# petabi/petal-neighbors

Measured on NVIDIA B200. Metric: knn_queries_per_sec_k10, higher is better.
Workload: dtype f32

## Files before the change

### petal-neighbors_b200/csrc/engine.cu

```cuda
#include <sys/mman.h>

#include <chrono>
#include <condition_variable>
#include <cstdio>
#include <cstdlib>
#include <memory>
#include <atomic>
#include <mutex>
#include <string>
#include <vector>

#include "../../include/petal_b200.h"
#include "flat_tree.hpp"
#include "comm.hpp"
#include "gpu_build.hpp"
#include "kernels.cuh"
#include "tc_filter.cuh"

namespace petal {

static thread_local std::string g_err;
static int fail(int code, const std::string& msg) {
    g_err = msg;
    return code;
// ... 456 lines not shown
        TRY(hb.ensure(sizeof(h)));
        CU(cudaMemcpyAsync(hb.p, &h, sizeof(h), cudaMemcpyHostToDevice, cm->stream));
        NC(cm->api->Broadcast(hb.p, hb.p, sizeof(h), ncclUint8, root, cm->comm, cm->stream));
        for (auto& a : replica_arrays()) NC(cm->api->Broadcast(a.first->p, a.first->p, a.second, ncclUint8, root, cm->comm, cm->stream));
        CU(cudaStreamSynchronize(cm->stream));
        return PN_OK;
    }
    int replicate_recv(pn_comm* cm, int root) {
        device = cm->device;
        DeviceGuard g(device);
        if (!g.ok) return fail(PN_CUDA, "cudaSetDevice failed");
        ReplicaHeader h{};
        DevBuf hb;
        TRY(hb.ensure(sizeof(h)));
        NC(cm->api->Broadcast(hb.p, hb.p, sizeof(h), ncclUint8, root, cm->comm, cm->stream));
        CU(cudaMemcpyAsync(&h, hb.p, sizeof(h), cudaMemcpyDeviceToHost, cm->stream));
        CU(cudaStreamSynchronize(cm->stream));
        ft.n = h.n; ft.n_total = h.n_total; ft.d = h.d; ft.dpad = h.dpad; ft.L = h.L; ft.n_internal = h.n_internal; ft.n_buckets = h.n_buckets;
        ft.n_nodes = h.n_nodes; ft.bucket_max = h.bucket_max; ft.kind = h.kind; kp = h.kp; algo = h.algo; tensor_ready = h.tensor_ready != 0;
        pmax = h.pmax; tscale = h.tscale; prune_on = (h.prune_on & 1u) != 0; tiles_on = (h.prune_on & 2u) != 0;
        gpu_built = true;
        bytes = 0;
        for (auto& a : replica_arrays()) {
            TRY(a.first->ensure(a.second));
            NC(cm->api->Broadcast(a.first->p, a.first->p, a.second, ncclUint8, root, cm->comm, cm->stream));
            bytes += a.first->cap;
        }
        CU(cudaStreamSynchronize(cm->stream));
        ft.bucket_lo.resize(ft.n_buckets); ft.bucket_hi.resize(ft.n_buckets);
        CU(cudaMemcpy(ft.bucket_lo.data(), d_blo.p, (size_t)ft.n_buckets * 4, cudaMemcpyDeviceToHost));
        CU(cudaMemcpy(ft.bucket_hi.data(), d_bhi.p, (size_t)ft.n_buckets * 4, cudaMemcpyDeviceToHost));
        if (ft.kind == 1) {
            ft.vp_ids.resize(std::max<uint32_t>(ft.n_nodes, 1));
            CU(cudaMemcpy(ft.vp_ids.data(), d_vpids.p, ft.vp_ids.size() * 4, cudaMemcpyDeviceToHost));
        }
        fill_dev_tree();
        return PN_OK;
    }
};

template <typename A>
struct Engine final : pn_tree {
    using V = typename VT<A>::V;
    std::shared_ptr<DeviceTree<A>> tree;
    bool owns_tree = true;
    int n_sms = 148;
    cudaStream_t stream = nullptr, last_stream = nullptr;
    cudaEvent_t ev[4] = {nullptr, nullptr, nullptr, nullptr};
    DevBuf w_qraw, w_q, w_home, w_hist, w_cursor, w_order, w_part_d, w_part_i, w_floor_d, w_floor_i,
        w_counters, w_out_i, w_out_d, w_counts, w_offsets, w_hits;
    cudaStream_t s_in = nullptr, s_out = nullptr;
    cudaEvent_t e_in[2] = {nullptr, nullptr}, e_cmp[2] = {nullptr, nullptr}, e_out[2] = {nullptr, nullptr};
    DevBuf w_qraw2[2], w_oi2[2], w_od2[2];
    DevBuf sh_li[2], sh_ld[2], sh_pack[2], sh_gat[2], sh_gat_d[2];
    std::vector<cudaEvent_t> sh_ev;
    DevBuf r_qraw[2], r_q[2], r_counts[2], r_offsets[2], r_hits[2], r_slab[2], r_qlist[2], r_nlist[2], r_sums[2];
    unsigned long long* pin_tot = nullptr;
    void* pin_stage[2] = {nullptr, nullptr};
    cudaEvent_t pin_ev[2] = {nullptr, nullptr};
    static constexpr size_t PIN_BYTES = 16u << 20;
    DevBuf w_aaug, w_qmargin, w_trace, w_gbound;
    bool last_used_tensor = false;
    DevBuf w_qs, w_seed, w_bits, w_tcnt;
    DevBuf w_bcen, w_brad, w_bmu, w_qth, w_bbits, w_bcnt, w_wslot, w_wlist, w_wbits, w_nwide;
    bool last_pruned = false, last_tiles = false;

    explicit Engine(std::shared_ptr<DeviceTree<A>> t) : tree(std::move(t)) {}
    ~Engine() override {
        if (!host_only) {
            DeviceGuard g(tree->device);
            for (auto& e : ev) if (e) cudaEventDestroy(e);
            for (int i = 0; i < 2; ++i) {
                if (pin_stage[i]) cudaFreeHost(pin_stage[i]);
                if (pin_ev[i]) cudaEventDestroy(pin_ev[i]);
                for (cudaEvent_t e : {e_in[i], e_cmp[i], e_out[i]}) if (e) cudaEventDestroy(e);
            }
            for (cudaEvent_t e : sh_ev) cudaEventDestroy(e);
            if (pin_tot) cudaFreeHost(pin_tot);
            if (s_in) cudaStreamDestroy(s_in);
            if (s_out) cudaStreamDestroy(s_out);
            if (stream) cudaStreamDestroy(stream);
        }
    }

    int open_device() {
        DeviceGuard g(tree->device);
        if (!g.ok) return fail(PN_CUDA, "no usable CUDA device (there is no CPU fallback)");
        CU(cudaDeviceGetAttribute(&n_sms, cudaDevAttrMultiProcessorCount, tree->device));
        CU(cudaStreamCreateWithFlags(&stream, cudaStreamNonBlocking));
        for (auto& e : ev) CU(cudaEventCreate(&e));
        return PN_OK;
    }

    uint64_t device_bytes() const override {
        if (!owns_tree) return 0;
        const auto p = tree->partition();
        return tree->bytes + (p ? p->bytes : 0);
    }

    template <int DVR, int K, int KIND>
    int launch_knn_t(const DeviceTree<A>& t, const KnnArgs<A>& a, dim3 grid, cudaStream_t st) {
        size_t smem = DVR < 0 ? 0 : 2 * TILE_BYTES + (DVR == 0 ? (size_t)TQ * t.ft.dpad * sizeof(A) : 0);
        auto kern = knn_tile_kernel<A, DVR, K, KIND>;
        if (smem > 32 * 1024) CU(cudaFuncSetAttribute(kern, cudaFuncAttributeMaxDynamicSharedMemorySize, (int)smem));
        kern<<<grid, TQ, smem, st>>>(a);
        CU(cudaGetLastError());
        return PN_OK;
    }
    template <int K, int KIND>
    int launch_knn_k(const DeviceTree<A>& t, const KnnArgs<A>& a, dim3 grid, cudaStream_t st) {
        switch (t.dt.dv) {
            case 1: return launch_knn_t<1, K, KIND>(t, a, grid, st);
            case 2: return launch_knn_t<2, K, KIND>(t, a, grid, st);
            case 4: return launch_knn_t<4, K, KIND>(t, a, grid, st);
            case 8: return launch_knn_t<8, K, KIND>(t, a, grid, st);
            default:
                if ((size_t)t.ft.dpad * sizeof(A) > 1024) return launch_knn_t<-1, K, KIND>(t, a, grid, st);
                return launch_knn_t<0, K, KIND>(t, a, grid, st);
        }
    }
    int launch_knn(const DeviceTree<A>& t, const KnnArgs<A>& a, dim3 grid, cudaStream_t st, bool k1) {
        if (t.ft.kind == 0) return k1 ? launch_knn_k<1, 0>(t, a, grid, st) : launch_knn_k<16, 0>(t, a, grid, st);
        return k1 ? launch_knn_k<1, 1>(t, a, grid, st) : launch_knn_k<16, 1>(t, a, grid, st);
    }


    typedef CUresult (*EncodeTiledFn)(CUtensorMap*, CUtensorMapDataType, cuuint32_t, void*, const cuuint64_t*, const cuuint64_t*,
                                      const cuuint32_t*, const cuuint32_t*, CUtensorMapInterleave, CUtensorMapSwizzle,
                                      CUtensorMapL2promotion, CUtensorMapFloatOOBfill);
    static EncodeTiledFn encode_fn() {
        static EncodeTiledFn fn = [] {
            void* p = nullptr;
            cudaDriverEntryPointQueryResult q;
            if (cudaGetDriverEntryPoint("cuTensorMapEncodeTiled", &p, cudaEnableDefault, &q) != cudaSuccess) { (void)cudaGetLastError(); p = nullptr; }
            return (EncodeTiledFn)p;
        }();
        return fn;
    }
    static int make_map(CUtensorMap* m, void* base, uint64_t rows, uint32_t box_rows, uint32_t kp) {
        EncodeTiledFn fn = encode_fn();
        if (!fn) return fail(PN_CUDA, "cuTensorMapEncodeTiled entry point not found");
        cuuint64_t dims[2] = {kp, rows};
        cuuint64_t strides[1] = {(cuuint64_t)kp * 2};
        cuuint32_t box[2] = {(cuuint32_t)tc::KC, (cuuint32_t)box_rows};
        cuuint32_t estr[2] = {1, 1};
        CUresult r = fn(m, CU_TENSOR_MAP_DATA_TYPE_FLOAT16, 2, base, dims, strides, box, estr, CU_TENSOR_MAP_INTERLEAVE_NONE,
                        CU_TENSOR_MAP_SWIZZLE_64B, CU_TENSOR_MAP_L2_PROMOTION_L2_256B, CU_TENSOR_MAP_FLOAT_OOB_FILL_NONE);
        if (r != CUDA_SUCCESS) return fail(PN_CUDA, "cuTensorMapEncodeTiled failed with code " + std::to_string((int)r));
        return PN_OK;
    }
    static constexpr size_t filter_fixed_smem(int mt, uint32_t k) {
        return 1024 + 1024 + (size_t)4 * mt * 192 * 4 + (size_t)4 * mt * k * 32 * 8;
    }
    template <int DVR, int K, int MT, int NACC, int SW = tc::BN>
    int launch_filter_t(const DeviceTree<A>& t, const CUtensorMap& map_a, const tc::FilterArgs& fa, cudaStream_t st) {
        if (fa.tile_bits) return launch_filter_s<DVR, K, MT, NACC, false, SW, true>(t, map_a, fa, st);
        return fa.g_bound ? launch_filter_s<DVR, K, MT, NACC, true, SW, false>(t, map_a, fa, st) : launch_filter_s<DVR, K, MT, NACC, false, SW, false>(t, map_a, fa, st);
    }
    template <int DVR, int K, int MT, int NACC, bool SHARED, int SW, bool PRUNE>
    int launch_filter_s(const DeviceTree<A>& t, const CUtensorMap& map_a, const tc::FilterArgs& fa, cudaStream_t st) {
        const size_t smem = filter_fixed_smem(MT, fa.k) + (size_t)MT * fa.nkc * tc::A_CHUNK_BYTES + (size_t)fa.stages * fa.gs * tc::CHUNK_BYTES;
        auto kern = tc::knn_filter_kernel<DVR, K, MT, NACC, SHARED, SW, PRUNE>;
        CU(cudaFuncSetAttribute(kern, cudaFuncAttributeMaxDynamicSharedMemorySize, (int)smem));
        const unsigned gx = (fa.nq - fa.row0 + MT * tc::BM - 1) / (MT * tc::BM);
        const unsigned gy = PRUNE ? 1u : (fa.n_tiles + fa.tiles_per_split - 1) / fa.tiles_per_split;
        kern<<<dim3(gx, gy), (5 * MT + 2) * 32, smem, st>>>(map_a, t.d_baug.template as<unsigned char>(), fa);
        CU(cudaGetLastError());
        return PN_OK;
    }
    template <int K>
    int launch_filter_k(const DeviceTree<A>& t, const CUtensorMap& map_a, tc::FilterArgs& fa, cudaStream_t st) {
        const int mt = t.filter_subtiles(fa.nkc);
        const size_t budget = 224 * 1024;
        fa.gs = fa.nkc == 1 ? 2 : (fa.nkc == 2 ? 2 : 1);
        const size_t fixed = filter_fixed_smem(mt, fa.k) + (size_t)mt * fa.nkc * tc::A_CHUNK_BYTES;
        fa.stages = fixed < budget ? (uint32_t)std::min<size_t>(fa.gs > 1 ? 8 : 12, (budget - fixed) / (tc::CHUNK_BYTES * fa.gs)) : 0;
        fa.stages &= ~1u;
        if (fa.stages < 2) return fail(PN_CUDA, "tensor path: shared memory budget too small for this dimension");
        if (mt == 4) {
            bool half = fa.nkc == 1;
#ifdef PN_TC_PROFILE
            if (getenv("PN_TC_HALF")) half = atoi(getenv("PN_TC_HALF")) != 0;
#endif
            if (half) {
                if (t.dt.dv == 4) return launch_filter_t<4, K, 4, 2, 64>(t, map_a, fa, st);
                if (t.dt.dv == 8) return launch_filter_t<8, K, 4, 2, 64>(t, map_a, fa, st);
                return launch_filter_t<0, K, 4, 2, 64>(t, map_a, fa, st);
            }
            if (t.dt.dv == 4) return launch_filter_t<4, K, 4, 1>(t, map_a, fa, st);
            if (t.dt.dv == 8) return launch_filter_t<8, K, 4, 1>(t, map_a, fa, st);
            return launch_filter_t<0, K, 4, 1>(t, map_a, fa, st);
        }
#if defined(PN_TC_PROFILE) || defined(PN_TC_EXPERIMENTS)
        if (mt == 3) {
            if (fa.nkc == 1) return t.dt.dv == 4 ? launch_filter_t<4, K, 3, 2, 64>(t, map_a, fa, st) : launch_filter_t<0, K, 3, 2, 64>(t, map_a, fa, st);
            return launch_filter_t<0, K, 3, 1>(t, map_a, fa, st);
        }
#endif
        if (mt == 2) {
            if (t.dt.dv == 4) return launch_filter_t<4, K, 2, 2>(t, map_a, fa, st);
            if (t.dt.dv == 8) return launch_filter_t<8, K, 2, 2>(t, map_a, fa, st);
#if defined(PN_TC_PROFILE) || defined(PN_TC_EXPERIMENTS)
            {
                static const int ts = getenv("PN_TC_TS") ? atoi(getenv("PN_TC_TS")) : 0;
                if (ts == 1 && fa.nkc <= 8) return launch_filter_t<0, K, 2, 2, 64>(t, map_a, fa, st);
                if (ts == 2) return launch_filter_t<0, K, 2, 1>(t, map_a, fa, st);
            }
#endif
            return launch_filter_t<0, K, 2, 2>(t, map_a, fa, st);
        }
        return launch_filter_t<0, K, 1, 2>(t, map_a, fa, st);
    }

    int sort_and_seed(const DeviceTree<A>& t, const A* qraw, uint32_t nq, size_t stride, uint32_t k, cudaStream_t st, bool self_query, const float4** qsorted,
                      const uint32_t** order) {
        if constexpr (sizeof(A) == 4) {
            *order = nullptr;
            TRY(w_home.ensure((size_t)nq * 4));
            if (self_query) {
                TRY(w_hist.ensure((size_t)t.ft.n_buckets * 4));
                home_bucket_kernel<A><<<(nq + 127) / 128, 128, 0, st>>>(t.dt, t.d_pts.template as<V>(), nq, w_home.as<uint32_t>(), w_hist.as<uint32_t>());
                CU(cudaGetLastError());
                ++counters.kernel_launches;
                *qsorted = t.d_pts.template as<float4>();
            } else {
                TRY(stage_queries(t, qraw, nq, stride, st, true));
                TRY(w_qs.ensure((size_t)nq * t.ft.dpad * 4));
                const size_t tot = (size_t)nq * t.dt.dv;
                tc::gather_queries_kernel<<<(unsigned)((tot + 255) / 256), 256, 0, st>>>(w_q.as<float4>(), w_order.as<uint32_t>(), nq, t.dt.dv, w_qs.as<float4>());
                CU(cudaGetLastError());
                ++counters.kernel_launches;
                *qsorted = w_qs.as<float4>();
                *order = w_order.as<uint32_t>();
            }
            TRY(w_seed.ensure((size_t)nq * 4));
            const DevTree<float>& dtf = *reinterpret_cast<const DevTree<float>*>(&t.dt);
            tc::seed_bound_kernel<<<(nq + 7) / 8, 256, 0, st>>>(dtf, *qsorted, *order, w_home.as<uint32_t>(), nq, k, w_seed.as<float>());
            CU(cudaGetLastError());
            ++counters.kernel_launches;
            return PN_OK;
        } else {
            (void)qraw; (void)nq; (void)stride; (void)k; (void)st; (void)self_query; (void)qsorted; (void)order;
            return fail(PN_BAD_ARG, "the tensor path is f32 only");
        }
    }

    int knn_device_pruned(const DeviceTree<A>& t, const A* qraw, uint32_t nq, size_t stride, uint32_t k, uint32_t kstride, uint64_t* idx_out, A* dist_out, cudaStream_t st,
                          bool self_query) {
        if constexpr (sizeof(A) == 4) {
            const bool k1 = (k == 1);
            const uint32_t KP = k1 ? 1 : 16;
            const uint32_t n_tiles = (uint32_t)((t.ft.n + tc::BN - 1) / tc::BN), words = (n_tiles + 31) / 32;
            const uint32_t QT = 128u * (uint32_t)t.filter_subtiles(t.kp / tc::KC), n_qt = (nq + QT - 1) / QT;
            const float4* qsorted;
            const uint32_t* order = nullptr;
            CU(cudaEventRecord(ev[2], st));
            static const bool stage_timing = getenv("PN_STAGE_TIMING") != nullptr;
            cudaEvent_t se[5] = {nullptr, nullptr, nullptr, nullptr, nullptr};
            if (stage_timing) { for (auto& e : se) CU(cudaEventCreate(&e)); CU(cudaEventRecord(se[0], st)); }
            TRY(sort_and_seed(t, qraw, nq, stride, k, st, self_query, &qsorted, &order));
            if (stage_timing) CU(cudaEventRecord(se[1], st));
            TRY(w_aaug.ensure((size_t)nq * t.kp * 2));
            TRY(w_qmargin.ensure((size_t)nq * 4));
            TRY(w_bits.ensure((size_t)n_qt * words * 4));
            TRY(w_tcnt.ensure((size_t)n_qt * 4));
            TRY(w_part_d.ensure((size_t)nq * KP * 4));
            TRY(w_part_i.ensure((size_t)nq * KP * 4));
            const DevTree<float>& dtf = *reinterpret_cast<const DevTree<float>*>(&t.dt);
            tc::build_aaug_kernel<<<(nq + 127) / 128, 128, 0, st>>>(reinterpret_cast<const float*>(qsorted), t.d_center.template as<float>(), t.tscale, nq, t.ft.d, t.ft.dpad,
                                                                    t.kp, t.pmax, w_aaug.as<__half>(), w_qmargin.as<float>());
            CU(cudaGetLastError());
            {
                static const int wide_div = getenv("PN_WIDE_DIV") ? atoi(getenv("PN_WIDE_DIV")) : 4;
                const uint32_t n_sub = QT / 32, n_warps = n_qt * n_sub, n_balls = 2 * n_warps;
                const uint32_t wide_cap = wide_div > 0 ? std::max<uint32_t>(1u, n_warps / (uint32_t)wide_div) : 1u;
                const size_t smem = (size_t)32 * t.dt.dv * 16;
                TRY(w_bcen.ensure((size_t)n_balls * t.ft.dpad * 4)); TRY(w_brad.ensure((size_t)n_balls * 4)); TRY(w_bmu.ensure((size_t)n_balls * 4));
                TRY(w_qth.ensure((size_t)n_warps * 32 * 4)); TRY(w_bbits.ensure((size_t)n_balls * words * 4)); TRY(w_bcnt.ensure((size_t)n_balls * 4));
                TRY(w_wslot.ensure((size_t)n_warps * 4)); TRY(w_wlist.ensure((size_t)wide_cap * 4)); TRY(w_wbits.ensure((size_t)wide_cap * words * 4));
                TRY(w_nwide.ensure(4));
                if (smem > 48u * 1024u) {
                    CU(cudaFuncSetAttribute(tc::ball_tile_kernel<false>, cudaFuncAttributeMaxDynamicSharedMemorySize, (int)smem));
                    CU(cudaFuncSetAttribute(tc::ball_tile_kernel<true>, cudaFuncAttributeMaxDynamicSharedMemorySize, (int)smem));
                }
                CU(cudaMemsetAsync(w_nwide.p, 0, 4, st));
                tc::warp_balls_kernel<<<(n_warps + 7) / 8, 256, 0, st>>>(qsorted, w_seed.as<float>(), nq, n_warps, t.dt.dv, w_bcen.as<float4>(), w_brad.as<float>(),
                                                                         w_bmu.as<float>(), w_qth.as<float>());
                CU(cudaGetLastError());
                tc::ball_tile_kernel<false><<<(n_balls + 31) / 32, 256, smem, st>>>(w_bcen.as<float4>(), w_brad.as<float>(), w_bmu.as<float>(), n_balls, nullptr, nullptr, 0u,
                                                                                   t.d_tcen.template as<float>(), t.d_trad.template as<float>(), n_tiles, t.dt.dv, (float)t.dt.slack, words,
                                                                                   w_bbits.as<uint32_t>(), w_bcnt.as<uint32_t>());
                CU(cudaGetLastError());
                tc::wide_select_kernel<<<(n_qt + 127) / 128, 128, 0, st>>>(w_bcnt.as<uint32_t>(), w_bmu.as<float>(), n_qt, n_sub, wide_div > 0 ? wide_cap : 0u, w_wslot.as<uint32_t>(),
                                                                          w_wlist.as<uint32_t>(), w_nwide.as<uint32_t>());
                CU(cudaGetLastError());
                tc::ball_tile_kernel<true><<<wide_cap, 256, smem, st>>>(qsorted, nullptr, w_qth.as<float>(), nq, w_wlist.as<uint32_t>(), w_nwide.as<uint32_t>(), wide_div > 0 ? wide_cap : 0u,
                                                                       t.d_tcen.template as<float>(), t.d_trad.template as<float>(), n_tiles, t.dt.dv, (float)t.dt.slack, words,
                                                                       w_wbits.as<uint32_t>(), nullptr);
                CU(cudaGetLastError());
                tc::group_bits_kernel<<<n_qt, 256, 0, st>>>(w_bbits.as<uint32_t>(), w_wbits.as<uint32_t>(), w_wslot.as<uint32_t>(), nq, QT, n_sub, words,
                                                            w_bits.as<uint32_t>(), w_tcnt.as<uint32_t>(), w_counters.as<unsigned long long>() + 3);
                CU(cudaGetLastError());
                counters.kernel_launches += 4;
            }
            counters.kernel_launches += 2;
            if (stage_timing) CU(cudaEventRecord(se[2], st));
            alignas(64) CUtensorMap map_a;
            TRY(make_map(&map_a, w_aaug.p, nq, tc::BM, t.kp));
            tc::FilterArgs fa{};
            fa.t = dtf;
            fa.q = qsorted; fa.q_margin = w_qmargin.as<float>();
            fa.k = k; fa.n_tiles = n_tiles; fa.tiles_per_split = n_tiles;
            fa.nkc = t.kp / tc::KC;
            fa.last_steps = ((t.ft.d + tc::NSLOT - 1) % tc::KC) / 16 + 1;
            fa.t2_scale = t.tscale * t.tscale * (1.0f + (float)(t.ft.d + 4) * 1.1920928955078125e-07f);
            fa.part_d = w_part_d.as<float>(); fa.part_i = w_part_i.as<uint32_t>();
            fa.counters = w_counters.as<unsigned long long>();
            fa.row0 = 0; fa.nq = nq; fa.g_bound = nullptr;
            fa.tile_bits = w_bits.as<uint32_t>(); fa.tile_cnt = w_tcnt.as<uint32_t>(); fa.tile_words = words; fa.seed_t2 = w_seed.as<float>();
            TRY(k1 ? launch_filter_k<1>(t, map_a, fa, st) : launch_filter_k<16>(t, map_a, fa, st));
            if (stage_timing) CU(cudaEventRecord(se[3], st));
            CU(merge_lists<A, uint32_t>(st, w_part_d.as<A>(), w_part_i.as<uint32_t>(), 1, nq, k, idx_out, dist_out, kstride,
                                                                            0, nullptr, nullptr, self_query ? t.d_ids.template as<uint32_t>() : order));
            CU(cudaGetLastError());
            if (stage_timing) {
                CU(cudaEventRecord(se[4], st));
                CU(cudaEventSynchronize(se[4]));
                float t[4] = {0.f, 0.f, 0.f, 0.f};
                for (int i = 0; i < 4; ++i) (void)cudaEventElapsedTime(&t[i], se[i], se[i + 1]);
                fprintf(stderr, "[pn stage timing] pruned scan, %u queries, k %u: sort + seeds %.2f ms | operands + tile bitmaps %.2f ms | filter %.2f ms | merge %.2f ms\n",
                        nq, k, t[0], t[1], t[2], t[3]);
                for (auto& e : se) cudaEventDestroy(e);
            }
            counters.kernel_launches += 2;
            counters.filter_pairs += (uint64_t)t.ft.n * nq;
            CU(cudaEventRecord(ev[3], st));
            return PN_OK;
        } else {
            (void)qraw; (void)nq; (void)stride; (void)k; (void)kstride; (void)idx_out; (void)dist_out; (void)st; (void)self_query;
            return fail(PN_BAD_ARG, "the tensor path is f32 only");
// ... 1526 lines not shown
```

### petal-neighbors_b200/csrc/tc_filter.cuh

```cuda
#pragma once
#include <cuda.h>
#include <cuda_fp16.h>
#include <cuda_runtime.h>
#include <stdint.h>

#include "kernels.cuh"
#include "tc_prune.cuh"

namespace petal {
namespace tc {

#ifdef PN_TC_PROFILE
#define PROF_DECL unsigned pt_ = (unsigned)clock(), pc_[6] = {0, 0, 0, 0, 0, 0}
#define PROF_ADD(i) do { unsigned n_ = (unsigned)clock(); pc_[i] += n_ - pt_; pt_ = n_; } while (0)
#define PROF_FLUSH(base) do { for (int i_ = 0; i_ < 6; ++i_) atomicAdd(&a.counters[8 + (base) + i_], (unsigned long long)pc_[i_]); } while (0)
#else
#define PROF_DECL
#define PROF_ADD(i)
#define PROF_FLUSH(base)
#endif
#if defined(PN_TC_PROFILE) && defined(PN_TC_TRACE)
#define TRACE(role, tile, ev) do { if (a.trace && blockIdx.x == 0 && (tile) >= a.trace_t0 && (tile) < a.trace_t0 + 64u) a.trace[(((role) * 64) + ((tile) - a.trace_t0)) * 4 + (ev)] = clock64(); } while (0)
#else
#define TRACE(role, tile, ev)
// ... 78 lines not shown
}
__host__ __device__ constexpr uint32_t make_idesc_f16(int M, int N) {
    return (1u << 4) | ((uint32_t)(N >> 3) << 17) | ((uint32_t)(M >> 4) << 24);
}

__device__ __forceinline__ void tmem_ld32_issue(uint32_t taddr, uint32_t (&r)[32]) {
    asm volatile(
        "tcgen05.ld.sync.aligned.32x32b.x32.b32 "
        "{%0, %1, %2, %3, %4, %5, %6, %7, %8, %9, %10, %11, %12, %13, %14, %15, "
        "%16, %17, %18, %19, %20, %21, %22, %23, %24, %25, %26, %27, %28, %29, %30, %31}, [%32];"
        : "=r"(r[0]), "=r"(r[1]), "=r"(r[2]), "=r"(r[3]), "=r"(r[4]), "=r"(r[5]), "=r"(r[6]), "=r"(r[7]), "=r"(r[8]),
          "=r"(r[9]), "=r"(r[10]), "=r"(r[11]), "=r"(r[12]), "=r"(r[13]), "=r"(r[14]), "=r"(r[15]), "=r"(r[16]),
          "=r"(r[17]), "=r"(r[18]), "=r"(r[19]), "=r"(r[20]), "=r"(r[21]), "=r"(r[22]), "=r"(r[23]), "=r"(r[24]),
          "=r"(r[25]), "=r"(r[26]), "=r"(r[27]), "=r"(r[28]), "=r"(r[29]), "=r"(r[30]), "=r"(r[31])
        : "r"(taddr)
        : "memory");
}
__device__ __forceinline__ void tmem_ld_wait(uint32_t (&r)[32]) {
    asm volatile("tcgen05.wait::ld.sync.aligned;"
                 : "+r"(r[0]), "+r"(r[1]), "+r"(r[2]), "+r"(r[3]), "+r"(r[4]), "+r"(r[5]), "+r"(r[6]), "+r"(r[7]), "+r"(r[8]),
                   "+r"(r[9]), "+r"(r[10]), "+r"(r[11]), "+r"(r[12]), "+r"(r[13]), "+r"(r[14]), "+r"(r[15]), "+r"(r[16]),
                   "+r"(r[17]), "+r"(r[18]), "+r"(r[19]), "+r"(r[20]), "+r"(r[21]), "+r"(r[22]), "+r"(r[23]), "+r"(r[24]),
                   "+r"(r[25]), "+r"(r[26]), "+r"(r[27]), "+r"(r[28]), "+r"(r[29]), "+r"(r[30]), "+r"(r[31])
                 :
                 : "memory");
}

struct SmemTopK {
    unsigned long long* sk;
    unsigned long long kth_key, floor_key;
    float t2;
    uint32_t k;
    static __device__ __forceinline__ unsigned long long make_key(float d, uint32_t i) {
        return ((unsigned long long)__float_as_uint(d) << 32) | i;
    }
    __device__ __forceinline__ void init(unsigned long long* base, int lane, uint32_t k_, bool active) {
        sk = base + lane; k = k_;
        kth_key = make_key(pos_inf<float>(), NO_ID);
        for (uint32_t s = 0; s < k; ++s) sk[s * 32] = kth_key;
        t2 = active ? pos_inf<float>() : -1.f;
        floor_key = 0ull;
    }
    __device__ __forceinline__ void set_floor(float d, uint32_t i) { floor_key = make_key(d, i) + 1ull; }
    __device__ __forceinline__ bool offer_key(unsigned long long key) {
        if (key < floor_key || key >= kth_key) return false;
        uint32_t p = k - 1;
        while (p > 0) {
            const unsigned long long pk = sk[(p - 1) * 32];
            if (key >= pk) break;
            sk[p * 32] = pk;
            --p;
        }
        sk[p * 32] = key;
        kth_key = sk[(k - 1) * 32];
        t2 = thresh2(__uint_as_float((uint32_t)(kth_key >> 32)));
        return true;
    }
    __device__ __forceinline__ void store(float* out_d, uint32_t* out_i) const {
        for (uint32_t s = 0; s < k; ++s) {
            const unsigned long long e = sk[s * 32];
            out_d[s] = __uint_as_float((uint32_t)(e >> 32)); out_i[s] = (uint32_t)e;
        }
    }
};

struct FilterArgs {
    DevTree<float> t;
    const float4* q;
    const float* q_margin;
    uint32_t nq, k;
    uint32_t row0;
    uint32_t n_tiles;
    uint32_t tiles_per_split;
    uint32_t nkc;
    uint32_t last_steps;
    uint32_t stages;
    uint32_t gs;
    float t2_scale;
    float* g_bound;
    float* part_d;
    uint32_t* part_i;
    const float* floor_d;
    const uint32_t* floor_i;
    unsigned long long* counters;
    const uint32_t* tile_bits;
    const uint32_t* tile_cnt;
    const float* seed_t2;
    uint32_t tile_words;
#ifdef PN_TC_PROFILE
    uint32_t dbg;
    long long* trace;
    uint32_t trace_t0;
#endif
};

__device__ __forceinline__ void split3_f16(float x, __half& h1, __half& h2, __half& h3) {
    h1 = __float2half_rn(x);
    const float r1 = x - __half2float(h1);
    h2 = __float2half_rn(r1);
    h3 = __float2half_rn(r1 - __half2float(h2));
}

__device__ __forceinline__ size_t baug_offset(uint32_t row, uint32_t j, uint32_t nkc) {
    const uint32_t tile = row / BN, r = row % BN, c = j / KC, e = j % KC;
    return ((size_t)(tile * nkc + c) * BN + r) * KC + (((e >> 3) ^ ((r >> 1) & 3u)) << 3) + (e & 7u);
}
__global__ void build_baug_kernel(const float* __restrict__ pts, const float* __restrict__ center, float scale, uint32_t n,
                                  uint32_t d, uint32_t dpad, uint32_t kp, __half* __restrict__ baug, unsigned int* pmax_bits) {
    const uint32_t i = blockIdx.x * blockDim.x + threadIdx.x;
    if (i >= n) return;
    const float* p = pts + (size_t)i * dpad;
    const uint32_t nkc = kp / KC;
    float nrm = 0.f;
    for (uint32_t j = 0; j < d; ++j) {
        const float v = (p[j] - center[j]) * scale;
        nrm = nrm + v * v;
        baug[baug_offset(i, j, nkc)] = __float2half_rn(-2.0f * v);
    }
    for (uint32_t j = d + NSLOT; j < kp; ++j) baug[baug_offset(i, j, nkc)] = __float2half_rn(0.f);
    __half h1, h2, h3;
    split3_f16(nrm, h1, h2, h3);
    const __half one = __float2half_rn(1.f);
    baug[baug_offset(i, d, nkc)] = one;     baug[baug_offset(i, d + 1, nkc)] = one; baug[baug_offset(i, d + 2, nkc)] = one;
    baug[baug_offset(i, d + 3, nkc)] = h1;  baug[baug_offset(i, d + 4, nkc)] = h2;  baug[baug_offset(i, d + 5, nkc)] = h3;
    atomicMax(pmax_bits, __float_as_uint(sqrtf(nrm) * 1.000001f));
}

__global__ void build_aaug_kernel(const float* __restrict__ q, const float* __restrict__ center, float scale, uint32_t nq,
                                  uint32_t d, uint32_t dpad, uint32_t kp, float pmax, __half* __restrict__ aaug,
                                  float* __restrict__ q_margin) {
    const uint32_t i = blockIdx.x * blockDim.x + threadIdx.x;
    if (i >= nq) return;
    const float* p = q + (size_t)i * dpad;
    __half* o = aaug + (size_t)i * kp;
    float nrm = 0.f;
    for (uint32_t j = 0; j < d; ++j) {
        const float v = (p[j] - center[j]) * scale;
        nrm = nrm + v * v;
    }
    const float qn = sqrtf(nrm) * 1.000001f;
    const bool in_range = qn <= 200.f;
    for (uint32_t j = 0; j < d; ++j) o[j] = __float2half_rn(in_range ? (p[j] - center[j]) * scale : 0.f);
    for (uint32_t j = d + NSLOT; j < kp; ++j) o[j] = __float2half_rn(0.f);
    __half h1, h2, h3;
    split3_f16(in_range ? nrm : 0.f, h1, h2, h3);
    const __half one = __float2half_rn(1.f);
    o[d] = h1; o[d + 1] = h2; o[d + 2] = h3; o[d + 3] = one; o[d + 4] = one; o[d + 5] = one;
    const float sn = qn + pmax;
    const float e = 1.01f * 0.001953125f * qn * pmax + 6.2e-05f * sqrtf((float)d) * (qn + 2.f * pmax) +
                    (float)(kp + 8) * 4.76837158203125e-07f * sn * sn;
    q_margin[i] = in_range ? e : pos_inf<float>();
}

template <int DVR, int K, int MT, int NUM_ACC, bool SHARED, int SW = BN, bool PRUNE = false>
__global__ void __launch_bounds__((5 * MT + 2) * 32, 1)
knn_filter_kernel(const __grid_constant__ CUtensorMap map_a, const unsigned char* __restrict__ baug, const FilterArgs a) {
    extern __shared__ __align__(1024) unsigned char smem_raw[];
    unsigned char* smem = (unsigned char*)(((uintptr_t)smem_raw + 1023) & ~(uintptr_t)1023);
    unsigned char* smem_a = smem;
    unsigned char* smem_b = smem + (size_t)MT * a.nkc * A_CHUNK_BYTES;
    uint64_t* bars = reinterpret_cast<uint64_t*>(smem_b + (size_t)a.stages * a.gs * CHUNK_BYTES);
    uint64_t* full_bar = bars;
    uint64_t* empty_bar = bars + a.stages;
    uint64_t* tfull_bar = bars + 2 * a.stages;
    uint64_t* tempty_bar = tfull_bar + NUM_ACC * MT;
    uint64_t* a_bar = tempty_bar + NUM_ACC * MT;
    uint32_t* tmem_slot = reinterpret_cast<uint32_t*>(a_bar + 1);
    uint32_t* qbuf = tmem_slot + 4;
    constexpr int QWORDS = 192;
    unsigned long long* tk = reinterpret_cast<unsigned long long*>(qbuf + 4 * MT * QWORDS);

    const int warp = __shfl_sync(0xffffffffu, threadIdx.x >> 5, 0), lane = threadIdx.x & 31;
    constexpr int EPI_WARPS = 4 * MT;
    constexpr bool TS = (MT == 2 && (NUM_ACC == 1 || SW == 64)) || MT == 3;
    constexpr int TMEM_COLS = TS ? 512 : NUM_ACC * MT * SW;
    constexpr int U = BN / SW;
    static_assert(SW == BN || SW == 64, "stage width is a whole tile or half a tile");

    if (warp == EPI_WARPS && lane == 0) {
        for (uint32_t s = 0; s < a.stages; ++s) { mbar_init(&full_bar[s], 1); mbar_init(&empty_bar[s], MT); }
        for (int s = 0; s < NUM_ACC * MT; ++s) { mbar_init(&tfull_bar[s], 1); mbar_init(&tempty_bar[s], 4); }
        mbar_init(a_bar, 1);
        asm volatile("fence.mbarrier_init.release.cluster;" ::: "memory");
        asm volatile("prefetch.tensormap [%0];" ::"l"(&map_a) : "memory");
    }
    if (warp == EPI_WARPS + 1) {
        asm volatile("tcgen05.alloc.cta_group::1.sync.aligned.shared::cta.b32 [%0], %1;" ::"r"(smem_u32(tmem_slot)), "r"(TMEM_COLS) : "memory");
        asm volatile("tcgen05.relinquish_alloc_permit.cta_group::1.sync.aligned;" ::: "memory");
    }
    tc_fence_before();
    __syncthreads();
    tc_fence_after();
    const uint32_t tmem_base = __shfl_sync(0xffffffffu, *tmem_slot, 0);

    const uint32_t row_base = a.row0 + blockIdx.x * (MT * BM);
    static_assert(!(PRUNE && SHARED), "the pruned scan does not split the point stream");
    const uint32_t j_begin = PRUNE ? 0u : blockIdx.y * a.tiles_per_split;
    const uint32_t n_my = PRUNE ? a.tile_cnt[blockIdx.x] : min(a.n_tiles - j_begin, a.tiles_per_split);
    const uint32_t* my_bits = PRUNE ? a.tile_bits + (size_t)blockIdx.x * a.tile_words : nullptr;

    if (warp == EPI_WARPS || warp == EPI_WARPS + MT + 1) {
        const uint32_t pid = warp == EPI_WARPS ? 0u : 1u;
        if (lane == 0) {
            if (pid == 0) {
                mbar_expect_tx(a_bar, (uint32_t)(MT * a.nkc * A_CHUNK_BYTES));
                for (int mt = 0; mt < MT; ++mt)
                    for (uint32_t c = 0; c < a.nkc; ++c)
                        tma_load_2d(&map_a, a_bar, smem_a + (size_t)(mt * a.nkc + c) * A_CHUNK_BYTES, (int)(c * KC), (int)(row_base + mt * BM));
            }
            const uint32_t total = n_my * a.nkc;
            const uint32_t n_groups = (total + a.gs - 1) / a.gs;
            const unsigned char* bsrc = baug + (size_t)j_begin * a.nkc * CHUNK_BYTES;
            PROF_DECL;
            if (PRUNE) {
                TileIter it;
                if (n_my) it.init(my_bits);
                for (uint32_t i = 0, ch = 0; i < n_my; ++i) {
                    const uint32_t tile = it.next();
                    for (uint32_t c = 0; c < a.nkc; ++c, ++ch) {
                        const uint32_t g = ch / a.gs, gi = ch % a.gs;
                        if ((g & 1u) != pid) continue;
                        const uint32_t s = g % a.stages, ph = (g / a.stages) & 1u;
                        if (gi == 0) {
                            mbar_wait(&empty_bar[s], ph ^ 1u);
                            mbar_expect_tx(&full_bar[s], min(a.gs, total - ch) * CHUNK_BYTES);
                        }
                        bulk_copy(smem_b + (size_t)(s * a.gs + gi) * CHUNK_BYTES, baug + ((size_t)tile * a.nkc + c) * CHUNK_BYTES, CHUNK_BYTES, &full_bar[s]);
                    }
                }
            } else
            for (uint32_t g = pid; g < n_groups; g += 2) {
                const uint32_t s = g % a.stages, ph = (g / a.stages) & 1u;
                const uint32_t first = g * a.gs, cnt = min(a.gs, total - first);
                PROF_ADD(1);
                mbar_wait(&empty_bar[s], ph ^ 1u);
                PROF_ADD(0);
#ifdef PN_TC_PROFILE
                if (a.dbg & 2u) { mbar_arrive(&full_bar[s]); continue; }
#endif
                mbar_expect_tx(&full_bar[s], cnt * CHUNK_BYTES);
                bulk_copy(smem_b + (size_t)s * a.gs * CHUNK_BYTES, bsrc + (size_t)first * CHUNK_BYTES, cnt * CHUNK_BYTES, &full_bar[s]);
            }
            if (pid == 0) PROF_FLUSH(12);
        }
    } else if (warp > EPI_WARPS && warp <= EPI_WARPS + MT) {
        {
            const int mt = warp - (EPI_WARPS + 1);
            const uint64_t a_desc0 = make_desc_sw64(smem_u32(smem_a)) + (uint64_t)(mt * a.nkc * (A_CHUNK_BYTES >> 4));
            const uint64_t b_desc0 = make_desc_sw64(smem_u32(smem_b));
            const uint32_t total = n_my * a.nkc;
            mbar_wait(a_bar, 0);
            const uint32_t a_ksteps = 2 * a.nkc - (a.last_steps > 1 ? 0u : 1u);
            const uint32_t a_tmem = tmem_base + NUM_ACC * MT * SW + mt * (a_ksteps * 8);
            if (TS) {
                tc_fence_after();
                if (elect_one()) {
                    for (uint32_t c = 0; c < a.nkc; ++c) {
                        const uint64_t ad = a_desc0 + (uint64_t)(c * (A_CHUNK_BYTES >> 4));
                        tc_cp_128x256b(a_tmem + c * 16, ad);
                        if (c + 1 < a.nkc || a.last_steps > 1) tc_cp_128x256b(a_tmem + c * 16 + 8, ad + 2);
                    }
                }
                __syncwarp();
            }
            uint32_t it = 0, g = 0, gi = 0, s = 0, sph = 0;
            uint32_t u = 0;
            constexpr uint32_t idesc_u = make_idesc_f16(BM, SW);
            PROF_DECL;
            for (uint32_t j = 0; j < n_my; ++j) {
                const uint32_t it0 = it, g0 = g, gi0 = gi, s0 = s, sph0 = sph;
#pragma unroll
                for (int h = 0; h < U; ++h, ++u) {
                    if (h) { it = it0; g = g0; gi = gi0; s = s0; sph = sph0; }
                    const uint32_t as = u % NUM_ACC, aph = (u / NUM_ACC) & 1u;
                    mbar_wait(&tempty_bar[as * MT + mt], aph ^ 1u);
                    tc_fence_after();
                    PROF_ADD(0);
                    if (lane == 0) TRACE(8 + mt, j, 0);
                    const uint32_t d_tmem = tmem_base + (as * MT + mt) * SW;
                    for (uint32_t c = 0; c < a.nkc; ++c, ++it) {
                        if (gi == 0 && h == 0) {
                            mbar_wait(&full_bar[s], sph);
                            tc_fence_after();
                            PROF_ADD(1);
                        }
                        if (lane == 0 && c == 0) TRACE(8 + mt, j, 1);
                        const uint64_t bd = b_desc0 + (uint64_t)((s * a.gs + gi) * (CHUNK_BYTES >> 4) + h * (SW * KC * 2 >> 4));
                        const uint64_t ad = a_desc0 + (uint64_t)(c * (A_CHUNK_BYTES >> 4));
                        const bool last = gi + 1 == a.gs || it + 1 == total;
                        if (elect_one()) {
                            const bool two = c + 1 < a.nkc || a.last_steps > 1;
                            if (TS) {
                                tc_mma_f16_ts(d_tmem, a_tmem + c * 16, bd, idesc_u, c > 0 ? 1u : 0u);
                                if (two) tc_mma_f16_ts(d_tmem, a_tmem + c * 16 + 8, bd + 2, idesc_u, 1u);
                            } else {
                                tc_mma_f16(d_tmem, ad, bd, idesc_u, c > 0 ? 1u : 0u);
                                if (two) tc_mma_f16(d_tmem, ad + 2, bd + 2, idesc_u, 1u);
                            }
                            if (last && h == U - 1) tc_commit(&empty_bar[s]);
                        }
                        __syncwarp();
                        if (last) { gi = 0; ++g; if (++s == a.stages) { s = 0; sph ^= 1u; } } else ++gi;
                    }
                    if (elect_one()) tc_commit(&tfull_bar[as * MT + mt]);
                    __syncwarp();
                    PROF_ADD(2);
                    if (lane == 0) TRACE(8 + mt, j, 2);
                }
            }
            if (mt == 0 && lane == 0) PROF_FLUSH(0);
        }
    } else {
        const int mt = warp >> 2, quad = warp & 3;
        const uint32_t wrow0 = row_base + mt * BM + quad * 32;
        const uint32_t qrow = wrow0 + lane;
        const bool active = qrow < a.nq;
        const DevTree<float>& t = a.t;
        const int DV = DVR > 0 ? DVR : (int)t.dv;
        unsigned long long* q_ent = reinterpret_cast<unsigned long long*>(qbuf + warp * QWORDS);
        unsigned long long* x_key = q_ent + 64;
        SmemTopK topk;
        topk.init(tk + warp * (a.k * 32), lane, a.k, active);
        if (a.floor_d && active) topk.set_floor(a.floor_d[qrow], a.floor_i[qrow]);
        const float margin = active ? a.q_margin[qrow] : 0.f;
        const float t2s = a.t2_scale;
        const float seed2 = a.seed_t2 && active ? a.seed_t2[qrow] : pos_inf<float>();
        TileIter titer;
        if (PRUNE && n_my) titer.init(my_bits);
        float theta = active ? xadd(xmul(seed2, t2s), margin) : -pos_inf<float>();
        float* gb = SHARED && active ? a.g_bound + (qrow - a.row0) : nullptr;
        auto refresh_theta = [&](bool publish) {
            float b = fminf(topk.t2, seed2);
            if (SHARED && gb) {
                if (publish) atomicMin(reinterpret_cast<int*>(gb), __float_as_int(b));
                b = fminf(b, __ldcg(gb));
            }
            theta = xadd(xmul(b, t2s), margin);
        };
        const unsigned full = 0xffffffffu;
        const unsigned lt_mask = (1u << lane) - 1u;
        unsigned long long hits = 0;
        int qn = 0;

        auto drain = [&](int cnt) {
            unsigned long long key = ~0ull;
            int o = 32 + lane;
            const bool valid = lane < cnt;
            if (valid) {
                const unsigned long long e = q_ent[lane];
                o = (int)(e >> 32);
                const uint32_t prow = (uint32_t)e;
                const float4* qr = a.q + (size_t)(wrow0 + o) * DV;
                const float4* pr = t.pts + (size_t)prow * DV;
                float acc = 0.f;
                if (DVR > 0) {
#pragma unroll
                    for (int jc = 0; jc < (DVR > 0 ? DVR : 1); ++jc) acc = fold(acc, __ldg(qr + jc), __ldg(pr + jc));
                } else {
                    for (int jc = 0; jc < DV; ++jc) acc = fold(acc, __ldg(qr + jc), __ldg(pr + jc));
                }
                key = SmemTopK::make_key(xsqrt(acc), __ldg(t.ids + prow));
            }
            const unsigned grp = __match_any_sync(full, o);
            const int rank = __popc(grp & lt_mask);
            const int rounds = __reduce_max_sync(full, valid ? rank + 1 : 0);
            for (int r = 0; r < rounds; ++r) {
                const bool send = valid && rank == r;
                if (send) x_key[o] = key;
                const unsigned owners = __reduce_or_sync(full, send ? (1u << o) : 0u);
                __syncwarp();
                if ((owners >> lane) & 1u) {
                    if (topk.offer_key(x_key[lane])) refresh_theta(true);
                }
                __syncwarp();
            }
        };

        auto test32 = [&](const uint32_t (&r)[32], uint32_t j, int col0, uint32_t& bits) -> bool {
            float mb[4];
#pragma unroll
            for (int b = 0; b < 4; ++b) {
                const float x0 = fminf(__uint_as_float(r[8 * b]), fminf(__uint_as_float(r[8 * b + 1]), __uint_as_float(r[8 * b + 2])));
                const float x1 = fminf(__uint_as_float(r[8 * b + 3]), fminf(__uint_as_float(r[8 * b + 4]), __uint_as_float(r[8 * b + 5])));
                mb[b] = fminf(fminf(x0, x1), fminf(__uint_as_float(r[8 * b + 6]), __uint_as_float(r[8 * b + 7])));
            }
            const float m = fminf(fminf(mb[0], mb[1]), fminf(mb[2], mb[3]));
            bits = 0;
            if (!__any_sync(full, m <= theta)) return false;
            if (m <= theta) {
#pragma unroll
                for (int b = 0; b < 4; ++b) {
                    if (mb[b] <= theta) {
#pragma unroll
                        for (int i = 0; i < 8; ++i) bits |= (__uint_as_float(r[8 * b + i]) <= theta ? 1u : 0u) << (8 * b + i);
                    }
                }
                const int valid = (int)t.n - (int)(j * BN + col0);
                if (valid < 32) bits &= valid > 0 ? ((1u << valid) - 1u) : 0u;
            }
            return true;
        };
        auto push32 = [&](uint32_t bits, uint32_t j, int col0) {
            for (;;) {
                const bool has = bits != 0;
                const unsigned mask = __ballot_sync(full, has);
                if (!mask) break;
                if (has) {
                    const int i = __ffs(bits) - 1;
                    bits &= bits - 1;
                    const int slot = qn + __popc(mask & lt_mask);
                    const uint32_t prow = j * BN + col0 + i;
                    q_ent[slot] = (unsigned long long)prow | ((unsigned long long)lane << 32);
                    asm volatile("prefetch.global.L2 [%0];" ::"l"(t.pts + (size_t)prow * DV));
                }
                qn += __popc(mask);
                hits += __popc(mask);
                __syncwarp();
                if (qn >= 32) {
                    drain(32);
                    const int rest = qn - 32;
                    unsigned long long te = 0;
                    if (lane < rest) te = q_ent[32 + lane];
                    __syncwarp();
                    if (lane < rest) q_ent[lane] = te;
                    __syncwarp();
                    qn = rest;
                }
            }
        };

        auto scan32 = [&](const uint32_t (&r)[32], uint32_t j, int col0) {
            float mb[4];
#pragma unroll
            for (int b = 0; b < 4; ++b) {
                const float x0 = fminf(__uint_as_float(r[8 * b]), fminf(__uint_as_float(r[8 * b + 1]), __uint_as_float(r[8 * b + 2])));
                const float x1 = fminf(__uint_as_float(r[8 * b + 3]), fminf(__uint_as_float(r[8 * b + 4]), __uint_as_float(r[8 * b + 5])));
                mb[b] = fminf(fminf(x0, x1), fminf(__uint_as_float(r[8 * b + 6]), __uint_as_float(r[8 * b + 7])));
            }
            const float m = fminf(fminf(mb[0], mb[1]), fminf(mb[2], mb[3]));
            if (!__any_sync(full, m <= theta)) return;
            uint32_t bits = 0;
            if (m <= theta) {
#pragma unroll
                for (int b = 0; b < 4; ++b) {
                    if (mb[b] <= theta) {
#pragma unroll
                        for (int i = 0; i < 8; ++i) bits |= (__uint_as_float(r[8 * b + i]) <= theta ? 1u : 0u) << (8 * b + i);
                    }
                }
                const int valid = (int)t.n - (int)(j * BN + col0);
                if (valid < 32) bits &= valid > 0 ? ((1u << valid) - 1u) : 0u;
            }
            for (;;) {
                const bool has = bits != 0;
                const unsigned mask = __ballot_sync(full, has);
                if (!mask) break;
                if (has) {
                    const int i = __ffs(bits) - 1;
                    bits &= bits - 1;
                    const int slot = qn + __popc(mask & lt_mask);
                    const uint32_t prow = j * BN + col0 + i;
                    q_ent[slot] = (unsigned long long)prow | ((unsigned long long)lane << 32);
                    asm volatile("prefetch.global.L2 [%0];" ::"l"(t.pts + (size_t)prow * DV));
// ... 168 lines not shown
```

Before: 9.538 million.

## Add lean filter variant with one MMA warp and one producer for nkc==1

Adds a LEAN template mode to the tensor-core filter kernel: a single MMA warp issues the MMAs for all MT subtiles, and a single TMA producer warp replaces the two alternating producers. This shrinks the block from 5*MT+2 to 4*MT+2 warps. With MT=4 and nkc==1 it replaces the previous half-width (SW=64, two accumulators) configuration with a full-width, single-accumulator lean kernel. The goal is to cut warp and barrier overhead, at the cost of serialising MMA issue across subtiles and losing accumulator double-buffering.

```diff
diff --git a/petal-neighbors_b200/csrc/engine.cu b/petal-neighbors_b200/csrc/engine.cu
--- a/petal-neighbors_b200/csrc/engine.cu
+++ b/petal-neighbors_b200/csrc/engine.cu
@@ -632,19 +632,20 @@
     static constexpr size_t filter_fixed_smem(int mt, uint32_t k) {
         return 1024 + 1024 + (size_t)4 * mt * 192 * 4 + (size_t)4 * mt * k * 32 * 8;
     }
-    template <int DVR, int K, int MT, int NACC, int SW = tc::BN>
+    template <int DVR, int K, int MT, int NACC, int SW = tc::BN, bool LEAN = false>
     int launch_filter_t(const DeviceTree<A>& t, const CUtensorMap& map_a, const tc::FilterArgs& fa, cudaStream_t st) {
-        if (fa.tile_bits) return launch_filter_s<DVR, K, MT, NACC, false, SW, true>(t, map_a, fa, st);
-        return fa.g_bound ? launch_filter_s<DVR, K, MT, NACC, true, SW, false>(t, map_a, fa, st) : launch_filter_s<DVR, K, MT, NACC, false, SW, false>(t, map_a, fa, st);
-    }
-    template <int DVR, int K, int MT, int NACC, bool SHARED, int SW, bool PRUNE>
+        if (fa.tile_bits) return launch_filter_s<DVR, K, MT, NACC, false, SW, true, LEAN>(t, map_a, fa, st);
+        return fa.g_bound ? launch_filter_s<DVR, K, MT, NACC, true, SW, false, LEAN>(t, map_a, fa, st)
+                          : launch_filter_s<DVR, K, MT, NACC, false, SW, false, LEAN>(t, map_a, fa, st);
+    }
+    template <int DVR, int K, int MT, int NACC, bool SHARED, int SW, bool PRUNE, bool LEAN>
     int launch_filter_s(const DeviceTree<A>& t, const CUtensorMap& map_a, const tc::FilterArgs& fa, cudaStream_t st) {
         const size_t smem = filter_fixed_smem(MT, fa.k) + (size_t)MT * fa.nkc * tc::A_CHUNK_BYTES + (size_t)fa.stages * fa.gs * tc::CHUNK_BYTES;
-        auto kern = tc::knn_filter_kernel<DVR, K, MT, NACC, SHARED, SW, PRUNE>;
+        auto kern = tc::knn_filter_kernel<DVR, K, MT, NACC, SHARED, SW, PRUNE, LEAN>;
         CU(cudaFuncSetAttribute(kern, cudaFuncAttributeMaxDynamicSharedMemorySize, (int)smem));
         const unsigned gx = (fa.nq - fa.row0 + MT * tc::BM - 1) / (MT * tc::BM);
         const unsigned gy = PRUNE ? 1u : (fa.n_tiles + fa.tiles_per_split - 1) / fa.tiles_per_split;
-        kern<<<dim3(gx, gy), (5 * MT + 2) * 32, smem, st>>>(map_a, t.d_baug.template as<unsigned char>(), fa);
+        kern<<<dim3(gx, gy), tc::filter_warps(MT, LEAN) * 32, smem, st>>>(map_a, t.d_baug.template as<unsigned char>(), fa);
         CU(cudaGetLastError());
         return PN_OK;
     }
@@ -658,14 +659,10 @@
         fa.stages &= ~1u;
         if (fa.stages < 2) return fail(PN_CUDA, "tensor path: shared memory budget too small for this dimension");
         if (mt == 4) {
-            bool half = fa.nkc == 1;
-#ifdef PN_TC_PROFILE
-            if (getenv("PN_TC_HALF")) half = atoi(getenv("PN_TC_HALF")) != 0;
-#endif
-            if (half) {
-                if (t.dt.dv == 4) return launch_filter_t<4, K, 4, 2, 64>(t, map_a, fa, st);
-                if (t.dt.dv == 8) return launch_filter_t<8, K, 4, 2, 64>(t, map_a, fa, st);
-                return launch_filter_t<0, K, 4, 2, 64>(t, map_a, fa, st);
+            if (fa.nkc == 1) {
+                if (t.dt.dv == 4) return launch_filter_t<4, K, 4, 1, tc::BN, true>(t, map_a, fa, st);
+                if (t.dt.dv == 8) return launch_filter_t<8, K, 4, 1, tc::BN, true>(t, map_a, fa, st);
+                return launch_filter_t<0, K, 4, 1, tc::BN, true>(t, map_a, fa, st);
             }
             if (t.dt.dv == 4) return launch_filter_t<4, K, 4, 1>(t, map_a, fa, st);
             if (t.dt.dv == 8) return launch_filter_t<8, K, 4, 1>(t, map_a, fa, st);
diff --git a/petal-neighbors_b200/csrc/tc_filter.cuh b/petal-neighbors_b200/csrc/tc_filter.cuh
--- a/petal-neighbors_b200/csrc/tc_filter.cuh
+++ b/petal-neighbors_b200/csrc/tc_filter.cuh
@@ -254,8 +254,10 @@
     q_margin[i] = in_range ? e : pos_inf<float>();
 }
 
-template <int DVR, int K, int MT, int NUM_ACC, bool SHARED, int SW = BN, bool PRUNE = false>
-__global__ void __launch_bounds__((5 * MT + 2) * 32, 1)
+__host__ __device__ constexpr int filter_warps(int mt, bool lean) { return lean ? 4 * mt + 2 : 5 * mt + 2; }
+
+template <int DVR, int K, int MT, int NUM_ACC, bool SHARED, int SW = BN, bool PRUNE = false, bool LEAN = false>
+__global__ void __launch_bounds__(filter_warps(MT, LEAN) * 32, 1)
 knn_filter_kernel(const __grid_constant__ CUtensorMap map_a, const unsigned char* __restrict__ baug, const FilterArgs a) {
     extern __shared__ __align__(1024) unsigned char smem_raw[];
     unsigned char* smem = (unsigned char*)(((uintptr_t)smem_raw + 1023) & ~(uintptr_t)1023);
@@ -274,13 +276,15 @@
 
     const int warp = __shfl_sync(0xffffffffu, threadIdx.x >> 5, 0), lane = threadIdx.x & 31;
     constexpr int EPI_WARPS = 4 * MT;
+    constexpr int NMMA = LEAN ? 1 : MT;
+    constexpr uint32_t NPROD = LEAN ? 1 : 2;
     constexpr bool TS = (MT == 2 && (NUM_ACC == 1 || SW == 64)) || MT == 3;
     constexpr int TMEM_COLS = TS ? 512 : NUM_ACC * MT * SW;
     constexpr int U = BN / SW;
     static_assert(SW == BN || SW == 64, "stage width is a whole tile or half a tile");
 
     if (warp == EPI_WARPS && lane == 0) {
-        for (uint32_t s = 0; s < a.stages; ++s) { mbar_init(&full_bar[s], 1); mbar_init(&empty_bar[s], MT); }
+        for (uint32_t s = 0; s < a.stages; ++s) { mbar_init(&full_bar[s], 1); mbar_init(&empty_bar[s], NMMA); }
         for (int s = 0; s < NUM_ACC * MT; ++s) { mbar_init(&tfull_bar[s], 1); mbar_init(&tempty_bar[s], 4); }
         mbar_init(a_bar, 1);
         asm volatile("fence.mbarrier_init.release.cluster;" ::: "memory");
@@ -301,7 +305,7 @@
     const uint32_t n_my = PRUNE ? a.tile_cnt[blockIdx.x] : min(a.n_tiles - j_begin, a.tiles_per_split);
     const uint32_t* my_bits = PRUNE ? a.tile_bits + (size_t)blockIdx.x * a.tile_words : nullptr;
 
-    if (warp == EPI_WARPS || warp == EPI_WARPS + MT + 1) {
+    if (warp == EPI_WARPS || (NPROD == 2 && warp == EPI_WARPS + NMMA + 1)) {
         const uint32_t pid = warp == EPI_WARPS ? 0u : 1u;
         if (lane == 0) {
             if (pid == 0) {
@@ -321,7 +325,7 @@
                     const uint32_t tile = it.next();
                     for (uint32_t c = 0; c < a.nkc; ++c, ++ch) {
                         const uint32_t g = ch / a.gs, gi = ch % a.gs;
-                        if ((g & 1u) != pid) continue;
+                        if (g % NPROD != pid) continue;
                         const uint32_t s = g % a.stages, ph = (g / a.stages) & 1u;
                         if (gi == 0) {
                             mbar_wait(&empty_bar[s], ph ^ 1u);
@@ -331,7 +335,7 @@
                     }
                 }
             } else
-            for (uint32_t g = pid; g < n_groups; g += 2) {
+            for (uint32_t g = pid; g < n_groups; g += NPROD) {
                 const uint32_t s = g % a.stages, ph = (g / a.stages) & 1u;
                 const uint32_t first = g * a.gs, cnt = min(a.gs, total - first);
                 PROF_ADD(1);
@@ -345,72 +349,82 @@
             }
             if (pid == 0) PROF_FLUSH(12);
         }
-    } else if (warp > EPI_WARPS && warp <= EPI_WARPS + MT) {
+    } else if (warp > EPI_WARPS && warp <= EPI_WARPS + NMMA) {
         {
-            const int mt = warp - (EPI_WARPS + 1);
-            const uint64_t a_desc0 = make_desc_sw64(smem_u32(smem_a)) + (uint64_t)(mt * a.nkc * (A_CHUNK_BYTES >> 4));
+            constexpr int MPW = MT / NMMA;
+            const int mt0 = (warp - (EPI_WARPS + 1)) * MPW;
+            const uint64_t a_desc00 = make_desc_sw64(smem_u32(smem_a));
             const uint64_t b_desc0 = make_desc_sw64(smem_u32(smem_b));
             const uint32_t total = n_my * a.nkc;
             mbar_wait(a_bar, 0);
             const uint32_t a_ksteps = 2 * a.nkc - (a.last_steps > 1 ? 0u : 1u);
-            const uint32_t a_tmem = tmem_base + NUM_ACC * MT * SW + mt * (a_ksteps * 8);
             if (TS) {
                 tc_fence_after();
                 if (elect_one()) {
-                    for (uint32_t c = 0; c < a.nkc; ++c) {
-                        const uint64_t ad = a_desc0 + (uint64_t)(c * (A_CHUNK_BYTES >> 4));
-                        tc_cp_128x256b(a_tmem + c * 16, ad);
-                        if (c + 1 < a.nkc || a.last_steps > 1) tc_cp_128x256b(a_tmem + c * 16 + 8, ad + 2);
+                    for (int m = 0; m < MPW; ++m) {
+                        const uint32_t a_tmem = tmem_base + NUM_ACC * MT * SW + (mt0 + m) * (a_ksteps * 8);
+                        for (uint32_t c = 0; c < a.nkc; ++c) {
+                            const uint64_t ad = a_desc00 + (uint64_t)(((mt0 + m) * a.nkc + c) * (A_CHUNK_BYTES >> 4));
+                            tc_cp_128x256b(a_tmem + c * 16, ad);
+                            if (c + 1 < a.nkc || a.last_steps > 1) tc_cp_128x256b(a_tmem + c * 16 + 8, ad + 2);
+                        }
                     }
                 }
                 __syncwarp();
             }
             uint32_t it = 0, g = 0, gi = 0, s = 0, sph = 0;
-            uint32_t u = 0;
             constexpr uint32_t idesc_u = make_idesc_f16(BM, SW);
             PROF_DECL;
             for (uint32_t j = 0; j < n_my; ++j) {
                 const uint32_t it0 = it, g0 = g, gi0 = gi, s0 = s, sph0 = sph;
 #pragma unroll
-                for (int h = 0; h < U; ++h, ++u) {
-                    if (h) { it = it0; g = g0; gi = gi0; s = s0; sph = sph0; }
-                    const uint32_t as = u % NUM_ACC, aph = (u / NUM_ACC) & 1u;
-                    mbar_wait(&tempty_bar[as * MT + mt], aph ^ 1u);
-                    tc_fence_after();
-                    PROF_ADD(0);
-                    if (lane == 0) TRACE(8 + mt, j, 0);
-                    const uint32_t d_tmem = tmem_base + (as * MT + mt) * SW;
-                    for (uint32_t c = 0; c < a.nkc; ++c, ++it) {
-                        if (gi == 0 && h == 0) {
-                            mbar_wait(&full_bar[s], sph);
-                            tc_fence_after();
-                            PROF_ADD(1);
+                for (int m = 0; m < MPW; ++m) {
+                    const int mt = mt0 + m;
+                    const uint64_t a_desc0 = a_desc00 + (uint64_t)(mt * a.nkc * (A_CHUNK_BYTES >> 4));
+                    const uint32_t a_tmem = tmem_base + NUM_ACC * MT * SW + mt * (a_ksteps * 8);
+#pragma unroll
+                    for (int h = 0; h < U; ++h) {
+                        const bool first = m == 0 && h == 0, final_u = m == MPW - 1 && h == U - 1;
+                        if (!first) { it = it0; g = g0; gi = gi0; s = s0; sph = sph0; }
+                        const uint32_t u = j * U + h;
+                        const uint32_t as = u % NUM_ACC, aph = (u / NUM_ACC) & 1u;
+                        mbar_wait(&tempty_bar[as * MT + mt], aph ^ 1u);
+                        tc_fence_after();
+                        PROF_ADD(0);
+                        if (lane == 0) TRACE(8 + mt, j, 0);
+                        const uint32_t d_tmem = tmem_base + (as * MT + mt) * SW;
+                        for (uint32_t c = 0; c < a.nkc; ++c, ++it) {
+                            if (gi == 0 && first) {
+                                mbar_wait(&full_bar[s], sph);
+                                tc_fence_after();
+                                PROF_ADD(1);
+                            }
+                            if (lane == 0 && c == 0) TRACE(8 + mt, j, 1);
+                            const uint64_t bd = b_desc0 + (uint64_t)((s * a.gs + gi) * (CHUNK_BYTES >> 4) + h * (SW * KC * 2 >> 4));
+                            const uint64_t ad = a_desc0 + (uint64_t)(c * (A_CHUNK_BYTES >> 4));
+                            const bool last = gi + 1 == a.gs || it + 1 == total;
+                            if (elect_one()) {
+                                const bool two = c + 1 < a.nkc || a.last_steps > 1;
+                                if (TS) {
+                                    tc_mma_f16_ts(d_tmem, a_tmem + c * 16, bd, idesc_u, c > 0 ? 1u : 0u);
+                                    if (two) tc_mma_f16_ts(d_tmem, a_tmem + c * 16 + 8, bd + 2, idesc_u, 1u);
+                                } else {
+                                    tc_mma_f16(d_tmem, ad, bd, idesc_u, c > 0 ? 1u : 0u);
+                                    if (two) tc_mma_f16(d_tmem, ad + 2, bd + 2, idesc_u, 1u);
+                                }
+                                if (last && final_u) tc_commit(&empty_bar[s]);
+                            }
+                            __syncwarp();
+                            if (last) { gi = 0; ++g; if (++s == a.stages) { s = 0; sph ^= 1u; } } else ++gi;
                         }
-                        if (lane == 0 && c == 0) TRACE(8 + mt, j, 1);
-                        const uint64_t bd = b_desc0 + (uint64_t)((s * a.gs + gi) * (CHUNK_BYTES >> 4) + h * (SW * KC * 2 >> 4));
-                        const uint64_t ad = a_desc0 + (uint64_t)(c * (A_CHUNK_BYTES >> 4));
-                        const bool last = gi + 1 == a.gs || it + 1 == total;
-                        if (elect_one()) {
-                            const bool two = c + 1 < a.nkc || a.last_steps > 1;
-                            if (TS) {
-                                tc_mma_f16_ts(d_tmem, a_tmem + c * 16, bd, idesc_u, c > 0 ? 1u : 0u);
-                                if (two) tc_mma_f16_ts(d_tmem, a_tmem + c * 16 + 8, bd + 2, idesc_u, 1u);
-                            } else {
-                                tc_mma_f16(d_tmem, ad, bd, idesc_u, c > 0 ? 1u : 0u);
-                                if (two) tc_mma_f16(d_tmem, ad + 2, bd + 2, idesc_u, 1u);
-                            }
-                            if (last && h == U - 1) tc_commit(&empty_bar[s]);
-                        }
+                        if (elect_one()) tc_commit(&tfull_bar[as * MT + mt]);
                         __syncwarp();
-                        if (last) { gi = 0; ++g; if (++s == a.stages) { s = 0; sph ^= 1u; } } else ++gi;
+                        PROF_ADD(2);
+                        if (lane == 0) TRACE(8 + mt, j, 2);
                     }
-                    if (elect_one()) tc_commit(&tfull_bar[as * MT + mt]);
-                    __syncwarp();
-                    PROF_ADD(2);
-                    if (lane == 0) TRACE(8 + mt, j, 2);
-                }
-            }
-            if (mt == 0 && lane == 0) PROF_FLUSH(0);
+                }
+            }
+            if (mt0 == 0 && lane == 0) PROF_FLUSH(0);
         }
     } else {
         const int mt = warp >> 2, quad = warp & 3;
```

New measurement: 8.931 million (median of 6 runs). -6.4%, worse.
